# FibonacciDude/ContrastiveProsthetics

Measured on AMD Instinct MI355X. Metric: sEMG windows/sec contrastive step, 12-ch Ninapro, 1/2/4/8 MI355X, higher is better.
Workload: dtype bf16; 1 GPU; synthetic 12-ch sEMG, 41-class one-hot, batch 4096 groups/GPU (167936 windows/GPU/step), stock BN (--no_adabn), dp_emg=0.0635, d_e=16, random-init weights; global_batch_groups=4096, parallelism=dp1, loss=reference per-group loss, tile_schedule=static

## Files before the change

contrastiveprosthetics_amd/csrc/api.hip:

```cpp
#include <hip/hip_runtime.h>
#include <cstdio>
#include <cmath>

#include "../../include/cpnative.h"
#include "common.cuh"
#include "gemm_nt.cuh"
#include "gemm_nt256p.cuh"
#include "gemm_ws.cuh"
#include "gemm_tn.cuh"
#include "gemm_tn256.cuh"
#include "kernels_misc.cuh"
#include "conv_kernels.cuh"
#include "head.cuh"
#include "optim.cuh"
#include "eval.cuh"
#include "preprocess.cuh"
#include "glove.cuh"
#include "fp8.cuh"
#include "small.cuh"
#include "online.cuh"
#include "online_adapt.cuh"
#include "online_multi.cuh"

static thread_local char g_err[512] = "";
// ... 266 lines not shown
    return 0;
}

extern "C" int cp_gather_oob_count(uint32_t* count_out, int32_t reset, void* stream) {
    if (!count_out) return fail(CP_ERR_ARG, "cp_gather_oob_count args");
    unsigned int* ctr = nullptr;
    CK(hipGetSymbolAddress((void**)&ctr, HIP_SYMBOL(g_gather_oob)));
    CK(hipMemcpyAsync(count_out, ctr, sizeof(uint32_t), hipMemcpyDeviceToDevice, (hipStream_t)stream));
    if (reset) CK(hipMemsetAsync(ctr, 0, sizeof(uint32_t), (hipStream_t)stream));
    return 0;
}

#define CAP_BDA16 512
#define CAP_BDA8 512
#define CAP_BRB16 512
#define CAP_BRB8 512
static inline int grid_rows(int64_t rows, int rows_per_block, int cap) {
    int64_t g = (rows + rows_per_block - 1) / rows_per_block;
    return (int)(g > cap ? cap : (g < 1 ? 1 : g));
}

template <typename T> static inline int fc_bm() { return sizeof(T) == 2 ? 256 : 128; }
template <typename T, int EPI>
static inline hipError_t launch_fc_gemm(const GemmNTArgs& a, hipStream_t st, int* stat_rows = nullptr, bool dyn_schedule = false) {
    if (stat_rows) *stat_rows = (int)((a.M + fc_bm<T>() - 1) / fc_bm<T>());
    if constexpr (sizeof(T) == 2) {
        const bool dyn = dyn_schedule, ws_ok = !dyn;
        if (EPI == EPI_FWD && a.K == WS_K && a.lda == WS_K && a.relu && ws_ok) return launch_gemm_ws(a, st, stat_rows);
        if (EPI == EPI_FWD && a.K == WSK_K && a.lda == WSK_K && a.F == 512 && a.relu && ws_ok) return launch_gemm_ws16n(a, st, stat_rows);
        if (EPI == EPI_FWD || (a.R == nullptr && a.dp_thresh == 0)) return launch_gemm_nt256p<EPI>(a, st, stat_rows, dyn);
        if (EPI == EPI_DGRAD && a.R != nullptr && a.K == WS_K && a.lda == WS_K && ws_ok) return launch_gemm_wsd_bn(a, st, stat_rows);
        if constexpr (EPI == EPI_DGRAD)
            return a.coef ? launch_gemm_nt256p<EPI_DGRAD_BN>(a, st, stat_rows, dyn) : launch_gemm_nt256p<EPI_DGRAD_ST>(a, st, stat_rows, dyn);
        return hipErrorInvalidValue;
    } else {
        return launch_gemm_nt<T, 128, 128, ALOAD_PLAIN, EPI>(a, st);
    }
}

template <typename T>
static inline int conv_grid(int64_t n_windows) {
    const int64_t strips = (n_windows + CONV_WPB - 1) / CONV_WPB;
    const int64_t cap = sizeof(T) == 2 ? 512 : 256;
    return (int)(strips < cap ? strips : cap);
}

struct PreReduce {
    const float* partials;
    float* scratch;
    hipStream_t st;
    const float* operator()(int& nrows, int W, int direct_rows = FIN_DIRECT_ROWS) const {
        if (nrows <= direct_rows) return partials;
        hipLaunchKernelGGL(reduce_rows_kernel, dim3(W / 64, REDUCE_SLICES), dim3(256), 0, st, partials, nrows, W, scratch);
        nrows = REDUCE_SLICES;
        return scratch;
    }
};

static int sync_row(const cp_config* c, const float* pp, int nrows, int width, unsigned char* base, const WS& w, hipStream_t st,
                    const float** glob, const float** local, const int* unscale_exp = nullptr) {
    float* loc = (float*)(base + w.sync_loc);
    float* glo = (float*)(base + w.sync_glob);
    if (width > 2 * 768) return fail(CP_ERR_ARG, "sync_row width");
    hipLaunchKernelGGL(colsum_finalize_kernel, dim3(FIN_GRID(width)), dim3(FIN_THREADS), 0, st, pp, nrows, width, loc, unscale_exp, width / 2);
    CKL("colsum_finalize_kernel(sync)");
    CK(hipMemcpyAsync(glo, loc, (size_t)width * 4, hipMemcpyDeviceToDevice, st));
    if (int e = c->stats_allreduce(c->stats_user, glo, width, st)) return fail(e, "the statistics all-reduce hook failed");
    *glob = glo;
    if (local) *local = loc;
    return 0;
}

template <typename T>
static int encoder_forward_t(const cp_config* c, const cp_params* p, const cp_bn_buffers* bn, const float* x,
                             unsigned char* base, const WS& w, float* z, hipStream_t st) {
    using D = DT<T>;
    const int64_t N = c->n_windows, R12 = N * 12;
    const bool batch_stats = c->training || c->adabn;
    const bool have_running = bn && bn->running_mean[0] && bn->running_var[0];
    if (!batch_stats && !have_running) return fail(CP_ERR_ARG, "eval with stock BN needs running statistics");
    const int upd = (c->training && !c->adabn && have_running) ? 1 : 0;
    const bool drop = c->training && c->dp_emg > 0.f;
    float* partials = (float*)(base + w.partials);
    auto act = [&](int l) { return (T*)(base + w.act[l]); };
    auto stats = [&](int l) { return (float*)(base + w.stats[l]); };
    auto finalize = [&](int l, int nrows, double count) -> int {
        if (!batch_stats) return 0;
        ProfScope ps(CP_K_BN_FINALIZE, st);
        const int C = kLayerC[l];
        const PreReduce pre{partials, (float*)(base + w.partials2), st};
        const float* pp = batch_stats ? pre(nrows, 2 * C) : partials;
        if (batch_stats && c->stats_allreduce) {
            if (int e = sync_row(c, pp, nrows, 2 * C, base, w, st, &pp, nullptr)) return e;
            nrows = 1;
            count *= c->stats_world;
        }
        hipLaunchKernelGGL(bn_finalize_kernel, dim3(FIN_GRID(C)), dim3(FIN_THREADS), 0, st, pp, nrows, count, p->bn_g[l], p->bn_b[l],
                           have_running ? bn->running_mean[l] : nullptr, have_running ? bn->running_var[l] : nullptr, upd,
                           batch_stats ? 0 : 1, c->bn_momentum, c->bn_eps, stats(l), C);
        hipError_t e = hipGetLastError();
        return e == hipSuccess ? 0 : fail((int)e, "bn_finalize_kernel");
    };

    {
        ProfScope ps(CP_K_PREP, st);
        hipLaunchKernelGGL((prep_conv2_kernel<T>), dim3(48), dim3(256), 0, st, p->conv2_w, (T*)(base + w.wc2_f), (T*)(base + w.wc2_d));
        CKL("prep_conv2_kernel");
        if (!batch_stats) {
            BnRunningAll ra{};
            for (int l = 0; l < CP_N_BN; ++l) {
                ra.gamma[l] = p->bn_g[l]; ra.beta[l] = p->bn_b[l]; ra.mean[l] = bn->running_mean[l]; ra.var[l] = bn->running_var[l];
                ra.stats[l] = stats(l); ra.C[l] = kLayerC[l];
            }
            ra.eps = c->bn_eps;
            hipLaunchKernelGGL(bn_running_stats_kernel, dim3(CP_N_BN), dim3(512), 0, st, ra);
            CKL("bn_running_stats_kernel");
            FoldBnBatch fb{};
            for (int i = 0; i < CP_N_FC; ++i) {
                const int Lp = 1 + i;
                fb.job[i] = FoldBnJob{p->fc_w[i], p->fc_b[i], stats(Lp) + 2 * kLayerC[Lp], stats(Lp) + 3 * kLayerC[Lp], base + w.wfc[i],
                                      (float*)(base + w.bfc[i]), 512, fcK(i), i == 0 ? 1 : 0, 512};
            }
            fb.job[CP_N_FC] = FoldBnJob{p->last_w, nullptr, stats(8) + 2 * 512, stats(8) + 3 * 512, base + w.wlast, (float*)(base + w.blast), CP_D_E, 512, 0, 32};
            hipLaunchKernelGGL((fold_linear_batch_kernel<T>), dim3(512, CP_N_FC + 1), dim3(256), 0, st, fb);
            CKL("fold_linear_batch_kernel");
        }
        if (drop) {
            FoldBatch fb{};
            for (int q = 0; q < 3; ++q)
                fb.job[q] = FoldJob{p->fc_w[4 + q], p->fc_b[4 + q], base + w.wfc[4 + q], (float*)(base + w.bfc[4 + q]), 512, 512, 512};
            fb.job[3] = FoldJob{p->last_w, nullptr, base + w.wlast, (float*)(base + w.blast), CP_D_E, 512, 32};
            hipLaunchKernelGGL((fold_copy_batch_kernel<T>), dim3(512, 4), dim3(256), 0, st, fb);
            CKL("fold_copy_batch_kernel");
        }
    }
    {
        constexpr int RPP = 256 / (64 / D::EPC);
        const int64_t need = (N + RPP - 1) / RPP, passes = (need + 2047) / 2048;
        const int g = (int)((need + passes - 1) / passes);
        if (batch_stats) {
            ProfScope ps(CP_K_CONV1_FWD, st);
            hipLaunchKernelGGL((conv1_stats_kernel<T>), dim3(g), dim3(256), 0, st, x, p->conv1_w, p->conv1_b, partials, R12);
            CKL("conv1_stats_kernel");
        }
        if (int e = finalize(0, g, (double)R12)) return e;
    }
    {
        ConvArgs ca{};
        ca.x = x; ca.w1 = p->conv1_w; ca.b1 = p->conv1_b; ca.stats1 = stats(0);
        ca.wc = base + w.wc2_f; ca.bias2 = p->conv2_b; ca.out = act(1); ca.partials = batch_stats ? partials : nullptr; ca.n_windows = N;
        const int g = conv_grid<T>(N);
        {
            ProfScope ps(CP_K_CONV2_FWD, st);
            hipLaunchKernelGGL((conv2_strip_kernel<T, 0>), dim3(g), dim3(256), 0, st, ca);
            CKL("conv2_strip_kernel<fwd>");
        }
        if (int e = finalize(1, g, (double)R12)) return e;
    }
    for (int i = 0; i < CP_N_FC; ++i) {
        const int L = 2 + i, Lp = L - 1, K = fcK(i);
        const T* A = act(Lp);
        const float *s = stats(Lp) + 2 * kLayerC[Lp], *t = stats(Lp) + 3 * kLayerC[Lp];
        if (drop && Lp >= 5) {
            T* u = (T*)(base + w.u[Lp - 5]);
            ProfScope ps(CP_K_DROPOUT, st);
            hipLaunchKernelGGL((bn_dropout_apply_kernel<T>), dim3(grid_rows(N, 256 / (512 / D::EPC), CAP_BDA16)), dim3(256), 0, st,
                               act(Lp), stats(Lp), u, N, 512, dp_thresh(c->dp_emg), dp_key(c, Lp), dp_inv_keep(c->dp_emg), dp_salt(c));
            CKL("bn_dropout_apply_kernel");
            A = u; s = nullptr; t = nullptr;
        }
        if (!(drop && Lp >= 5) && batch_stats) {
            ProfScope ps(CP_K_FOLD, st);
            hipLaunchKernelGGL((fold_linear_kernel<T>), dim3(512), dim3(256), 0, st, p->fc_w[i], p->fc_b[i], s, t,
                               (T*)(base + w.wfc[i]), (float*)(base + w.bfc[i]), 512, K, i == 0 ? 1 : 0);
            CKL("fold_linear_kernel");
        }
        GemmNTArgs a{};
        a.A = A; a.lda = K; a.M = N; a.K = K;
        a.W = base + w.wfc[i]; a.F = 512;
        a.C = act(L); a.ldc = 512; a.bias = (float*)(base + w.bfc[i]); a.relu = 1;
        a.partials = (batch_stats || sizeof(T) != 2 || dyn_tiles(c)) ? partials : nullptr;
        int nrows = 0;
        {
            const bool ws = sizeof(T) == 2 && K == WS_K && !dyn_tiles(c);
            ProfScope ps(ws ? CP_K_FC_FWD_WS : CP_K_FC_FWD, st);
            CK((launch_fc_gemm<T, EPI_FWD>(a, st, &nrows, dyn_tiles(c))));
        }
        if (int e = finalize(L, nrows, (double)N)) return e;
    }
    {
        const int Lp = 8;
        const T* A = act(Lp);
        const float *s = stats(Lp) + 2 * 512, *t = stats(Lp) + 3 * 512;
        if (!drop && batch_stats) {
            ProfScope ps(CP_K_FOLD, st);
            hipLaunchKernelGGL((fold_linear_kernel<T>), dim3(32), dim3(256), 0, st, p->last_w, (const float*)nullptr, s, t,
                               (T*)(base + w.wlast), (float*)(base + w.blast), CP_D_E, 512, 0);
            CKL("fold_linear_kernel(last)");
        }
        GemmNTArgs a{};
        a.A = A; a.lda = 512; a.M = N; a.K = 512;
        a.W = base + w.wlast; a.F = 32;
        a.C = z; a.ldc = CP_D_E; a.f_valid = CP_D_E; a.bias = (float*)(base + w.blast);
        {
            ProfScope ps(CP_K_PROJ_FWD, st);
            if (drop) {
                a.a_scale = stats(Lp) + 2 * 512; a.a_shift = stats(Lp) + 3 * 512;
                a.dp_thresh = dp_thresh(c->dp_emg); a.dp_key = dp_key(c, Lp); a.dp_inv_keep = dp_inv_keep(c->dp_emg); a.dp_salt = dp_salt(c);
                CK((launch_gemm_nt<T, 128, 32, ALOAD_BNDROP, EPI_PLAIN_F32>(a, st)));
            } else {
                CK((launch_gemm_nt<T, 128, 32, ALOAD_PLAIN, EPI_PLAIN_F32>(a, st)));
            }
        }
    }
    return 0;
}


static int encoder_forward_fp8(const cp_config* c, const cp_params* p, const cp_bn_buffers* bn, const float* x,
                               unsigned char* base, const WS& w, float* z, hipStream_t st) {
    using T = bf16_t;
    using D = DT<T>;
    const int64_t N = c->n_windows, R12 = N * 12;
    const bool batch_stats = c->training || c->adabn;
    const bool have_running = bn && bn->running_mean[0] && bn->running_var[0];
    if (!batch_stats && !have_running) return fail(CP_ERR_ARG, "eval with stock BN needs running statistics");
    const int upd = (c->training && !c->adabn && have_running) ? 1 : 0;
    const bool drop = c->training && c->dp_emg > 0.f;
    float* partials = (float*)(base + w.partials);
    Fp8State* fs = (Fp8State*)(base + w.f8state);
    auto stats = [&](int l) { return (float*)(base + w.stats[l]); };
    auto finalize = [&](int l, int nrows, double count, const int* unscale) -> int {
        if (!batch_stats) return 0;
        ProfScope ps(CP_K_BN_FINALIZE, st);
        const int C = kLayerC[l];
        const PreReduce pre{partials, (float*)(base + w.partials2), st};
        const float* pp = batch_stats ? pre(nrows, 2 * C) : partials;
        if (batch_stats && c->stats_allreduce) {
            if (int e = sync_row(c, pp, nrows, 2 * C, base, w, st, &pp, nullptr, unscale)) return e;
            nrows = 1;
            count *= c->stats_world;
            unscale = nullptr;
        }
        hipLaunchKernelGGL(bn_finalize_kernel, dim3(FIN_GRID(C)), dim3(FIN_THREADS), 0, st, pp, nrows, count, p->bn_g[l], p->bn_b[l],
                           have_running ? bn->running_mean[l] : nullptr, have_running ? bn->running_var[l] : nullptr, upd,
                           batch_stats ? 0 : 1, c->bn_momentum, c->bn_eps, stats(l), C, unscale);
        hipError_t e = hipGetLastError();
        return e == hipSuccess ? 0 : fail((int)e, "bn_finalize_kernel");
    };
    {
        ProfScope ps(CP_K_PREP, st);
        hipLaunchKernelGGL(fp8_update_scales_kernel, dim3(1), dim3(64), 0, st, fs, N);
        hipLaunchKernelGGL((prep_conv2_kernel<T>), dim3(48), dim3(256), 0, st, p->conv2_w, (T*)(base + w.wc2_f), (T*)(base + w.wc2_d));
        if (!batch_stats) {
            BnRunningAll ra{};
            for (int l = 0; l < CP_N_BN; ++l) {
                ra.gamma[l] = p->bn_g[l]; ra.beta[l] = p->bn_b[l]; ra.mean[l] = bn->running_mean[l]; ra.var[l] = bn->running_var[l];
                ra.stats[l] = stats(l); ra.C[l] = kLayerC[l];
            }
            ra.eps = c->bn_eps;
            hipLaunchKernelGGL(bn_running_stats_kernel, dim3(CP_N_BN), dim3(512), 0, st, ra);
        }
        if (batch_stats && drop) {
            Fold8Batch fb{};
            for (int i = 4; i < CP_N_FC; ++i)
                fb.job[i - 4] = Fold8Job{p->fc_w[i], p->fc_b[i], nullptr, nullptr, base + w.wfc8[i], base + w.wsc8[i],
                                         (float*)(base + w.bfc[i]), fcK(i), 0, F8_T_U + (i - 4), F8_T_ACT + 2 + i};
            hipLaunchKernelGGL(fold_linear8_batch_kernel, dim3(512, CP_N_FC - 4), dim3(256), 0, st, fb, (const Fp8State*)fs);
        }
        CKL("prep kernels (fp8)");
    }
    {
        constexpr int RPP = 256 / (64 / D::EPC);
        const int64_t need = (N + RPP - 1) / RPP, passes = (need + 2047) / 2048;
        const int g = (int)((need + passes - 1) / passes);
        if (batch_stats) {
            ProfScope ps(CP_K_CONV1_FWD, st);
            hipLaunchKernelGGL((conv1_stats_kernel<T>), dim3(g), dim3(256), 0, st, x, p->conv1_w, p->conv1_b, partials, R12);
            CKL("conv1_stats_kernel");
        }
        if (int e = finalize(0, g, (double)R12, nullptr)) return e;
    }
    {
        ConvArgs ca{};
        ca.x = x; ca.w1 = p->conv1_w; ca.b1 = p->conv1_b; ca.stats1 = stats(0);
        ca.wc = base + w.wc2_f; ca.bias2 = p->conv2_b; ca.out = nullptr; ca.partials = batch_stats ? partials : nullptr; ca.n_windows = N;
        ca.out8 = base + w.act8[1]; ca.out_exp = &fs->e[F8_T_ACT + 1]; ca.out_amax = &fs->amax[F8_T_ACT + 1];
        const int g = conv_grid<T>(N);
        {
            ProfScope ps(CP_K_CONV2_FWD, st);
            hipLaunchKernelGGL((conv2_strip_kernel<T, 0>), dim3(g), dim3(256), 0, st, ca);
            CKL("conv2_strip_kernel<fwd, e4m3>");
        }
        if (int e = finalize(1, g, (double)R12, nullptr)) return e;
    }
    if (!batch_stats) {
        ProfScope ps(CP_K_FOLD, st);
        Fold8Batch fb{};
        for (int i = 0; i < CP_N_FC; ++i) {
            const int Lp = 1 + i;
            fb.job[i] = Fold8Job{p->fc_w[i], p->fc_b[i], stats(Lp) + 2 * kLayerC[Lp], stats(Lp) + 3 * kLayerC[Lp], base + w.wfc8[i], base + w.wsc8[i],
                                 (float*)(base + w.bfc[i]), fcK(i), i == 0 ? 1 : 0, F8_T_ACT + Lp, F8_T_ACT + 2 + i};
        }
        hipLaunchKernelGGL(fold_linear8_batch_kernel, dim3(512, CP_N_FC), dim3(256), 0, st, fb, (const Fp8State*)fs);
        CKL("fold_linear8_batch_kernel");
    }
    for (int i = 0; i < CP_N_FC; ++i) {
// ... 2120 lines not shown
```

contrastiveprosthetics_amd/csrc/conv_kernels.cuh:

```cuda
#pragma once
#include <type_traits>
#include "common.cuh"
#include "gemm_tn.cuh"

#define CONV_WPB 16
#define CONV_ROWS (CONV_WPB * 12)
#define CONV_IMG_ROWS (CONV_WPB * 14)

struct ConvArgs {
    const float* x;
    const float* w1;
    const float* b1;
    const float* stats1;
    const void* wc;
    const float* bias2;
    const void* gin;
    const int* gin_exp;
    const float* coef;
    void* out;
    uint8_t* out8;
    const int* out_exp;
    uint32_t* out_amax;
    float* partials;
    int64_t n_windows;
    SmBN bn1;
    long long* acc_out;
    const float* bn2_rows;
    int bn2_nr;
    const void* r2;
    const float* stats2;
    float* dgamma2;
    float* dbeta2;
    float* gcols3;
    const float* rows1;
    int rows1_nr;
    float* dgamma1;
    float* dbeta1;
};

__device__ __forceinline__ void conv_bn_bwd_coef(const float* __restrict__ rows, int nr, int nfold, const float* __restrict__ stats, double count,
                                                 float* ca, float* cb, float* cz, double (*red)[4][64], bool writer, float* dgamma, float* dbeta) {
    const int tid = threadIdx.x, c = tid & 63, part = tid >> 6, W = nfold * 64;
    double s1 = 0, s2 = 0;
    const int total = nr * nfold;
    int i = part;
    for (; i + 28 < total; i += 32) {
        float v1[8], v2[8];
#pragma unroll
        for (int u = 0; u < 8; ++u) {
            const int k = i + 4 * u, rw = k / nfold, f = k % nfold;
            v1[u] = rows[((int64_t)rw * 2 + 0) * W + f * 64 + c];
            v2[u] = rows[((int64_t)rw * 2 + 1) * W + f * 64 + c];
        }
#pragma unroll
        for (int u = 0; u < 8; ++u) { s1 += (double)v1[u]; s2 += (double)v2[u]; }
    }
    for (; i < total; i += 4) {
        const int rw = i / nfold, f = i % nfold;
        s1 += (double)rows[((int64_t)rw * 2 + 0) * W + f * 64 + c];
        s2 += (double)rows[((int64_t)rw * 2 + 1) * W + f * 64 + c];
    }
    red[0][part][c] = s1;
    red[1][part][c] = s2;
    __syncthreads();
    if (tid < 64) {
        s1 = (red[0][0][c] + red[0][1][c]) + (red[0][2][c] + red[0][3][c]);
        s2 = (red[1][0][c] + red[1][1][c]) + (red[1][2][c] + red[1][3][c]);
        const double mean = stats[c], invstd = stats[64 + c], sc = stats[128 + c];
        const double dot = (s2 - mean * s1) * invstd;
        const double c1 = s1 / count, c2 = dot / count;
        ca[c] = (float)sc;
        cb[c] = (float)(-sc * invstd * c2);
        cz[c] = (float)(-sc * (c1 - mean * invstd * c2));
        if (writer) { dgamma[c] = (float)dot; dbeta[c] = (float)s1; }
    }
    __syncthreads();
}

template <typename T> struct ConvGeo {
    using D = DT<T>;
    static constexpr int EPC = D::EPC;
    static constexpr int CPR = 64 / EPC;
    static constexpr int ROWB = 64 * (int)sizeof(T);
    static constexpr int RPP = 256 / CPR;
    static constexpr int WPITCH = 192 * (int)sizeof(T) + 16;
    static constexpr int CPITCH = ROWB + 16;
    __device__ static __forceinline__ int swz(int row) {
        const int d = row - 2 * (row / 14);
        return sizeof(T) == 2 ? ((d >> 1) & 7) : (d & 15);
    }
    __device__ static __forceinline__ int img_off(int row, int chunk) { return row * ROWB + ((chunk ^ swz(row)) << 4); }
};

template <typename T>
__device__ __forceinline__ void conv1_chunk_vals(float xm, float x0, float xp, const float (*wt)[3], const float* bs, float* out) {
    using D = DT<T>;
    const f32x2_t xm2 = {xm, xm}, x02 = {x0, x0}, xp2 = {xp, xp};
#pragma unroll
    for (int e = 0; e < D::EPC; e += 2) {
        f32x2_t y = {bs[e], bs[e + 1]};
        y = __builtin_elementwise_fma((f32x2_t){wt[e][0], wt[e + 1][0]}, xm2, y);
        y = __builtin_elementwise_fma((f32x2_t){wt[e][1], wt[e + 1][1]}, x02, y);
        y = __builtin_elementwise_fma((f32x2_t){wt[e][2], wt[e + 1][2]}, xp2, y);
        if constexpr (sizeof(T) == 2) {
            const uint32_t pk = cvt_pk_bf16<true>(y.x, y.y);
            out[e] = __uint_as_float(pk << 16);
            out[e + 1] = __uint_as_float(pk & 0xffff0000u);
        } else {
            out[e] = fmaxf(y.x, 0.f);
            out[e + 1] = fmaxf(y.y, 0.f);
        }
    }
}
template <typename T>
__device__ __forceinline__ void conv1_chunk_row(const float* xr, int w, const float (*wt)[3], const float* bs, float* out) {
    const float x0 = xr[w];
    const float xl = xr[w > 0 ? w - 1 : 0];
    const float xh = xr[w < 11 ? w + 1 : 11];
    conv1_chunk_vals<T>(w > 0 ? xl : 0.f, x0, w < 11 ? xh : 0.f, wt, bs, out);
}
template <typename T>
__device__ __forceinline__ void conv1_chunk(const float* __restrict__ x, int64_t win, int w, const float (*wt)[3],
                                            const float* bs, float* out) {
    conv1_chunk_row<T>(x + win * 12, w, wt, bs, out);
}

template <typename T>
__global__ __launch_bounds__(256) void conv1_stats_kernel(const float* __restrict__ x, const float* __restrict__ w,
                                                          const float* __restrict__ bias, float* __restrict__ partials,
                                                          int64_t rows, long long* __restrict__ acc = nullptr) {
    using G = ConvGeo<T>;
    constexpr int EPC = G::EPC, CPR = G::CPR, RPP = G::RPP;
    __shared__ float red[2][RPP][64];
    const int tid = threadIdx.x, cc = tid % CPR, rr = tid / CPR;
    float wt[EPC][3], bs[EPC];
    f32x2_t s1[EPC / 2], s2[EPC / 2];
#pragma unroll
    for (int e = 0; e < EPC; ++e) {
#pragma unroll
        for (int k = 0; k < 3; ++k) wt[e][k] = w[(cc * EPC + e) * 9 + 3 + k];
        bs[e] = bias[cc * EPC + e];
    }
#pragma unroll
    for (int k = 0; k < EPC / 2; ++k) s1[k] = s2[k] = (f32x2_t){0.f, 0.f};
    const int64_t nwin = rows / 12;
    for (int64_t win = (int64_t)blockIdx.x * RPP + rr; win < nwin; win += (int64_t)gridDim.x * RPP) {
        float xv[12];
#pragma unroll
        for (int q = 0; q < 3; ++q) {
            const float4 t = *(const float4*)(x + win * 12 + 4 * q);
            xv[4 * q] = t.x; xv[4 * q + 1] = t.y; xv[4 * q + 2] = t.z; xv[4 * q + 3] = t.w;
        }
#pragma unroll
        for (int w = 0; w < 12; ++w) {
            float v[EPC];
            conv1_chunk_vals<T>(w > 0 ? xv[w - 1] : 0.f, xv[w], w < 11 ? xv[w + 1] : 0.f, wt, bs, v);
// ... 106 lines not shown
    auto prefetch_g = [&](int64_t strip) {
        if constexpr (MODE == 1) {
#pragma unroll
            for (int it = 0; it < NITG; ++it) {
                const int ir = rr + it * RPP;
                const int nl = ir / 14, wp = ir % 14;
                const int64_t win = strip * CONV_WPB + nl;
                const bool ok = strip < nstrips && wp >= 1 && wp <= 12 && win < a.n_windows;
                pg[it] = *(const uint4*)((const T*)a.gin + ((ok ? win : 0) * 12 + (ok ? wp - 1 : 0)) * 64 + cc * EPC);
            }
        }
    };
    prefetch_g(blockIdx.x);
    __syncthreads();
    for (int64_t strip = blockIdx.x; strip < nstrips; strip += gridDim.x) {
        const int64_t win0 = strip * CONV_WPB;
        const float x_next = MODE == 0 ? load_x(strip + gridDim.x) : 0.f;
        const float* xcur = xs[MODE == 0 ? xb : 0];
        {
            constexpr int NIT = CONV_IMG_ROWS / RPP;
            uint4 v[NIT];
#pragma unroll
            for (int it = 0; it < NIT; ++it) {
                const int ir = rr + it * RPP;
                const int nl = ir / 14, wp = ir % 14;
                const int64_t win = win0 + nl;
                const bool ok = wp >= 1 && wp <= 12 && win < a.n_windows;
                const int64_t winc = ok ? win : 0;
                const int wpos = ok ? wp - 1 : 0;
                if constexpr (MODE == 0) {
                    float t[EPC];
                    conv1_chunk_row<T>(xcur + nl * 12, wpos, wt, bs, t);
#pragma unroll
                    for (int e = 0; e < EPC; ++e) t[e] = fmaf(t[e], sc[e], sh[e]);
                    v[it] = D::pack(t);
                } else {
                    v[it] = pg[it];
                }
                if (!ok) v[it] = make_uint4(0, 0, 0, 0);
            }
#pragma unroll
            for (int it = 0; it < NIT; ++it) *(uint4*)(img + G::img_off(rr + it * RPP, cc)) = v[it];
        }
        __syncthreads();
        prefetch_g(strip + gridDim.x);
        f32x16 acc[3];
#pragma unroll
        for (int j = 0; j < 3; ++j)
#pragma unroll
            for (int g = 0; g < 16; ++g) acc[j][g] = 0.f;
        int ir0[3];
#pragma unroll
        for (int j = 0; j < 3; ++j) {
            const int ml = (st0 + j) * 32 + r;
            ir0[j] = (ml / 12) * 14 + (ml % 12);
        }
#pragma unroll
        for (int ks = 0; ks < NKS; ++ks) {
            const int tap = ks / KS_PER_TAP, chunk = (ks % KS_PER_TAP) * 2 + h;
            const uint4 fw = *(const uint4*)(Wl + (ft * 32 + r) * WPITCH + ks * 32 + h * 16);
#pragma unroll
            for (int j = 0; j < 3; ++j) {
                const uint4 fs = *(const uint4*)(img + G::img_off(ir0[j] + tap, chunk));
                mma_chunk<T>(fw, fs, acc[j]);
            }
        }
        if (MODE == 0 && tid < CONV_WPB * 12) xs[xb ^ 1][tid] = x_next;
        __syncthreads();
#pragma unroll
        for (int j = 0; j < 3; ++j) {
            const int srow = (st0 + j) * 32 + r;
#pragma unroll
            for (int q = 0; q < 4; ++q) {
                const int fl = ft * 32 + 8 * q + 4 * h;
                f32x2_t v0 = {acc[j][4 * q], acc[j][4 * q + 1]}, v1 = {acc[j][4 * q + 2], acc[j][4 * q + 3]};
                if constexpr (MODE == 0) {
                    v0 += (f32x2_t){b2v[q][0], b2v[q][1]};
                    v1 += (f32x2_t){b2v[q][2], b2v[q][3]};
                }
                unsigned char* dst = Cs + srow * CPITCH + fl * (int)sizeof(T);
                if constexpr (sizeof(T) == 2) {
                    *(uint2*)dst = make_uint2(cvt_pk_bf16<MODE == 0>(v0.x, v0.y), cvt_pk_bf16<MODE == 0>(v1.x, v1.y));
                } else {
                    if constexpr (MODE == 0) { v0 = __builtin_elementwise_max(v0, (f32x2_t){0.f, 0.f}); v1 = __builtin_elementwise_max(v1, (f32x2_t){0.f, 0.f}); }
                    *(float4*)dst = make_float4(v0.x, v0.y, v1.x, v1.y);
                }
            }
        }
        __syncthreads();
#pragma unroll
        for (int p = 0; p < CONV_ROWS / RPP; ++p) {
            const int row = rr + p * RPP;
            const int64_t m = win0 * 12 + row;
            const bool ok = m < total_rows;
            const int64_t mc = ok ? m : 0;
            const uint4 c = *(const uint4*)(Cs + row * CPITCH + cc * 16);
            float v[EPC];
            D::unpack(ok ? c : make_uint4(0, 0, 0, 0), v);
            if constexpr (MODE == 0) {
                if (want_sums) {
#pragma unroll
                    for (int k = 0; k < EPC / 2; ++k) {
                        const f32x2_t vp = {v[2 * k], v[2 * k + 1]};
                        s1[k] += vp;
                        s2[k] = __builtin_elementwise_fma(vp, vp, s2[k]);
                    }
                }
            } else {
                float r1[EPC];
                conv1_chunk<T>(a.x, mc / 12, (int)(mc % 12), wt, bs, r1);
#pragma unroll
                for (int k = 0; k < EPC / 2; ++k) {
                    const f32x2_t vp = {v[2 * k], v[2 * k + 1]}, rp = {r1[2 * k], r1[2 * k + 1]};
                    s1[k] += vp;
                    s2[k] = __builtin_elementwise_fma(vp, rp, s2[k]);
                }
            }
            if constexpr (MODE == 0 && sizeof(T) == 2) {
                if (a.out8 != nullptr) {
                    float w8[EPC];
#pragma unroll
                    for (int e = 0; e < EPC; ++e) { w8[e] = v[e] * out_scale; out_max = fmaxf(out_max, w8[e]); }
                    int p0 = __builtin_amdgcn_cvt_pk_fp8_f32(w8[0], w8[1], 0, false), p1 = __builtin_amdgcn_cvt_pk_fp8_f32(w8[4], w8[5], 0, false);
                    p0 = __builtin_amdgcn_cvt_pk_fp8_f32(w8[2], w8[3], p0, true);
                    p1 = __builtin_amdgcn_cvt_pk_fp8_f32(w8[6], w8[7], p1, true);
                    if (ok) *(uint2*)(a.out8 + m * 64 + cc * EPC) = make_uint2((uint32_t)p0, (uint32_t)p1);
                    continue;
                }
            }
            if (ok) *(uint4*)((T*)a.out + m * 64 + cc * EPC) = c;
        }
        __syncthreads();
        xb ^= 1;
    }
    if constexpr (MODE == 0 && sizeof(T) == 2) {
        if (a.out8 != nullptr) {
            out_max = wave_max(out_max);
            if ((tid & 63) == 0 && out_max > 0.f && __float_as_uint(out_max) > __hip_atomic_load(a.out_amax, __ATOMIC_RELAXED, __HIP_MEMORY_SCOPE_AGENT))
                atomicMax(a.out_amax, __float_as_uint(out_max));
        }
    }
#pragma unroll
    for (int e = 0; e < EPC; ++e) { red[(0 * RPP + rr) * 64 + cc * EPC + e] = s1[e / 2][e & 1]; red[(1 * RPP + rr) * 64 + cc * EPC + e] = s2[e / 2][e & 1]; }
    __syncthreads();
    if (tid < 128 && want_sums) {
        const int which = tid >> 6, c = tid & 63;
        float s = 0.f;
        for (int q = 0; q < RPP; ++q) s += red[(which * RPP + q) * 64 + c];
        if (MODE == 0 && a.acc_out != nullptr) sm_acc_add(a.acc_out + which * 64 + c, s, SM_ACT_SHIFT);
        else a.partials[((int64_t)blockIdx.x * 2 + which) * 64 + c] = s;
    }
}

#define CONV_WG_WPB 8
#define CONV_WG_IMG (CONV_WG_WPB * 14)
template <typename T, bool G8 = false, bool BN2 = false>
__global__ __launch_bounds__(256, BN2 ? 1 : 2) void conv2_wgrad_kernel(ConvArgs a) {
    static_assert(!G8 || sizeof(T) == 2, "e5m2 gradients are expanded into a bf16 image");
    static_assert(!(G8 && BN2), "the small-batch form reads T gradients");
    using GV = std::conditional_t<G8, uint2, uint4>;
    using D = DT<T>;
    using G = ConvGeo<T>;
    constexpr int EPC = G::EPC, CPR = G::CPR, RPP = G::RPP, KSTEP = D::KSTEP;
    constexpr int PITCH = TNPitch<T, 64>::value;
    constexpr int ROWS = CONV_WG_IMG + 2;
    constexpr int NIT = (CONV_WG_IMG + RPP - 1) / RPP;
    __shared__ __attribute__((aligned(16))) unsigned char smem[2 * ROWS * PITCH];
    unsigned char* Xi = smem;
    unsigned char* Yi = smem + ROWS * PITCH;
    const int tid = threadIdx.x, lane = tid & 63, wave = tid >> 6;
    const int cc = tid % CPR, rr = tid / CPR;
    const int ot = wave & 1, it = wave >> 1;
    const int64_t nstrips = (a.n_windows + CONV_WG_WPB - 1) / CONV_WG_WPB;

    float wt[EPC][3], bs[EPC], sc[EPC], sh[EPC];
#pragma unroll
    for (int e = 0; e < EPC; ++e) {
        const int c = cc * EPC + e;
#pragma unroll
        for (int k = 0; k < 3; ++k) wt[e][k] = a.w1[c * 9 + 3 + k];
        bs[e] = a.b1[c];
        sc[e] = a.stats1 ? a.stats1[2 * 64 + c] : 1.f;
        sh[e] = a.stats1 ? a.stats1[3 * 64 + c] : 0.f;
    }
    f32x16 acc[3];
#pragma unroll
    for (int j = 0; j < 3; ++j)
#pragma unroll
        for (int g = 0; g < 16; ++g) acc[j][g] = 0.f;
    uint4 xr2[BN2 ? NIT : 1];
    float c2a[BN2 ? EPC : 1], c2b[BN2 ? EPC : 1], c2z[BN2 ? EPC : 1], cs_all[BN2 ? EPC : 1], cs_first[BN2 ? EPC : 1], cs_last[BN2 ? EPC : 1];
    if constexpr (BN2) {
        __shared__ float ca_s[64], cb_s[64], cz_s[64];
        conv_bn_bwd_coef(a.bn2_rows, a.bn2_nr, 12, a.stats2, (double)a.n_windows * 12, ca_s, cb_s, cz_s, (double (*)[4][64])smem, blockIdx.x == 0,
                         a.dgamma2, a.dbeta2);
#pragma unroll
        for (int e = 0; e < EPC; ++e) {
            c2a[e] = ca_s[cc * EPC + e]; c2b[e] = cb_s[cc * EPC + e]; c2z[e] = cz_s[cc * EPC + e];
            cs_all[e] = cs_first[e] = cs_last[e] = 0.f;
        }
        __syncthreads();
    }
    if (rr == 0) {
        *(uint4*)(Xi + 0 * PITCH + cc * 16) = make_uint4(0, 0, 0, 0);
        *(uint4*)(Xi + (ROWS - 1) * PITCH + cc * 16) = make_uint4(0, 0, 0, 0);
        *(uint4*)(Yi + 0 * PITCH + cc * 16) = make_uint4(0, 0, 0, 0);
        *(uint4*)(Yi + (ROWS - 1) * PITCH + cc * 16) = make_uint4(0, 0, 0, 0);
    }
    GV xg[NIT];
    float xr[NIT][3];
    float gd = 1.f;
    if constexpr (G8) gd = f8_exp2i(-*a.gin_exp);
    auto prefetch = [&](int64_t strip) {
        const int64_t win0 = strip * CONV_WG_WPB;
#pragma unroll
        for (int q = 0; q < NIT; ++q) {
            const int ir = rr + q * RPP;
            const int nl = ir / 14, wp = ir % 14;
            const int64_t win = win0 + nl;
            const bool ok = strip < nstrips && ir < CONV_WG_IMG && wp >= 1 && wp <= 12 && win < a.n_windows;
            const int64_t winc = ok ? win : 0;
            const int wpos = ok ? wp - 1 : 0;
            xg[q] = *(const GV*)((const unsigned char*)a.gin + ((winc * 12 + wpos) * 64 + cc * EPC) * (int64_t)sizeof(GV) / EPC);
            if constexpr (BN2) xr2[q] = *(const uint4*)((const T*)a.r2 + (winc * 12 + wpos) * 64 + cc * EPC);
            const float* xw = a.x + winc * 12;
            xr[q][0] = xw[wpos > 0 ? wpos - 1 : 0];
            xr[q][1] = xw[wpos];
            xr[q][2] = xw[wpos < 11 ? wpos + 1 : 11];
        }
    };
    prefetch(blockIdx.x);
    for (int64_t strip = blockIdx.x; strip < nstrips; strip += gridDim.x) {
        const int64_t win0 = strip * CONV_WG_WPB;
        {
#pragma unroll
            for (int q = 0; q < NIT; ++q) {
                const int ir = rr + q * RPP;
                const int nl = ir / 14, wp = ir % 14;
                const bool ok = ir < CONV_WG_IMG && wp >= 1 && wp <= 12 && win0 + nl < a.n_windows;
                const int wpos = ok ? wp - 1 : 0;
                float t[EPC];
                conv1_chunk_vals<T>(wpos > 0 ? xr[q][0] : 0.f, xr[q][1], wpos < 11 ? xr[q][2] : 0.f, wt, bs, t);
                if (a.stats1 != nullptr) {
#pragma unroll
                    for (int e = 0; e < EPC; ++e) t[e] = fmaf(t[e], sc[e], sh[e]);
                }
                uint4 yv = D::pack(t);
                uint4 xv;
                if constexpr (G8) xv = f8_chunk5_to_bf16(xg[q], gd);
                else xv = xg[q];
                if constexpr (BN2) {
                    float gv[EPC], rv[EPC];
                    D::unpack(xv, gv);
                    D::unpack(xr2[q], rv);
#pragma unroll
                    for (int e = 0; e < EPC; ++e) gv[e] = rv[e] > 0.f ? fmaf(c2a[e], gv[e], fmaf(c2b[e], rv[e], c2z[e])) : 0.f;
                    xv = D::pack(gv);
                    if (ok) {
                        *(uint4*)((T*)const_cast<void*>(a.gin) + ((win0 + nl) * 12 + wpos) * 64 + cc * EPC) = xv;
                        D::unpack(xv, gv);
#pragma unroll
                        for (int e = 0; e < EPC; ++e) {
                            cs_all[e] += gv[e];
                            cs_first[e] += wpos == 0 ? gv[e] : 0.f;
                            cs_last[e] += wpos == 11 ? gv[e] : 0.f;
                        }
                    }
                }
                if (!ok) { xv = make_uint4(0, 0, 0, 0); yv = make_uint4(0, 0, 0, 0); }
                if (ir < CONV_WG_IMG) {
                    *(uint4*)(Xi + (ir + 1) * PITCH + cc * 16) = xv;
                    *(uint4*)(Yi + (ir + 1) * PITCH + cc * 16) = yv;
                }
            }
        }
        __syncthreads();
        prefetch(strip + gridDim.x);
#pragma unroll
        for (int k0 = 0; k0 < CONV_WG_IMG; k0 += KSTEP) {
            uint4 fy;
            if constexpr (sizeof(T) == 2) fy = tn_frag_bf16<PITCH>(Yi, k0 + 1, it * 32, lane);
            else fy = tn_frag_f32<PITCH>(Yi, k0 + 1, it * 32, lane);
#pragma unroll
            for (int tap = 0; tap < 3; ++tap) {
                uint4 fx;
                if constexpr (sizeof(T) == 2) fx = tn_frag_bf16<PITCH>(Xi, k0 + 2 - tap, ot * 32, lane);
                else fx = tn_frag_f32<PITCH>(Xi, k0 + 2 - tap, ot * 32, lane);
                mma_chunk<T>(fx, fy, acc[tap]);
            }
        }
        __syncthreads();
    }
    float* slab = a.partials + (int64_t)blockIdx.x * 64 * 192;
    const int r = lane & 31, h = lane >> 5;
#pragma unroll
    for (int tap = 0; tap < 3; ++tap) {
        const int q = tap * 64 + it * 32 + r;
#pragma unroll
        for (int g = 0; g < 16; ++g) {
            const int p = ot * 32 + (g & 3) + 8 * (g >> 2) + 4 * h;
            slab[p * 192 + q] = acc[tap][g];
        }
    }
    if constexpr (BN2) {
        float* red = (float*)smem;
        static_assert(2 * ROWS * PITCH >= 3 * RPP * 64 * 4, "the column-sum reduction reuses the image region");
// ... 168 lines not shown
```

Before: 47.39 million windows/s.

## Add software-pipelined conv2 forward kernel double-buffering the conv1 image build

Adds a new 16-bit conv2 forward kernel that loops persistently over strips. It builds the next strip's conv1+BN image into a second LDS buffer while the MFMA chains for the current strip run, and uses sched_group_barrier hints to interleave the two. Weights stay in registers, batch-stat sums are kept in registers and reduced once at the end, and outputs are stored through buffer stores. The aim is to hide LDS image construction and global loads behind matrix work, at the cost of higher register and LDS pressure and a more complex schedule.

```diff
diff --git a/contrastiveprosthetics_amd/csrc/api.hip b/contrastiveprosthetics_amd/csrc/api.hip
--- a/contrastiveprosthetics_amd/csrc/api.hip
+++ b/contrastiveprosthetics_amd/csrc/api.hip
@@ -442,7 +442,12 @@
         const int g = conv_grid<T>(N);
         {
             ProfScope ps(CP_K_CONV2_FWD, st);
-            hipLaunchKernelGGL((conv2_strip_kernel<T, 0>), dim3(g), dim3(256), 0, st, ca);
+            if constexpr (sizeof(T) == 2) {
+                if (batch_stats) hipLaunchKernelGGL((conv2_fwd_pipe_kernel<T, true>), dim3(g), dim3(256), 0, st, ca);
+                else hipLaunchKernelGGL((conv2_fwd_pipe_kernel<T, false>), dim3(g), dim3(256), 0, st, ca);
+            } else {
+                hipLaunchKernelGGL((conv2_strip_kernel<T, 0>), dim3(g), dim3(256), 0, st, ca);
+            }
             CKL("conv2_strip_kernel<fwd>");
         }
         if (int e = finalize(1, g, (double)R12)) return e;
diff --git a/contrastiveprosthetics_amd/csrc/conv_kernels.cuh b/contrastiveprosthetics_amd/csrc/conv_kernels.cuh
--- a/contrastiveprosthetics_amd/csrc/conv_kernels.cuh
+++ b/contrastiveprosthetics_amd/csrc/conv_kernels.cuh
@@ -2,6 +2,7 @@
 #include <type_traits>
 #include "common.cuh"
 #include "gemm_tn.cuh"
+#include "gemm_ws.cuh"
 
 #define CONV_WPB 16
 #define CONV_ROWS (CONV_WPB * 12)
@@ -414,6 +415,195 @@
     }
 }
 
+typedef __attribute__((ext_vector_type(2))) unsigned int u32x2_t;
+template <typename T, bool SUMS>
+__global__ __launch_bounds__(256, 2) void conv2_fwd_pipe_kernel(ConvArgs a) {
+    static_assert(sizeof(T) == 2, "the pipelined forward is the 16-bit large-batch form");
+    using D = DT<T>;
+    using G = ConvGeo<T>;
+    constexpr int EPC = G::EPC, CPR = G::CPR, ROWB = G::ROWB, RPP = G::RPP;
+    constexpr int KSTEP = D::KSTEP, KS_PER_TAP = 64 / KSTEP, NKS = 3 * KS_PER_TAP;
+    constexpr int IMG_BYTES = CONV_IMG_ROWS * ROWB, NIT = CONV_IMG_ROWS / RPP, XN = CONV_WPB * 12;
+    static_assert(2 * IMG_BYTES >= 2 * 64 * 64 * 4, "the end-of-kernel reduction reuses the image buffers");
+    __shared__ __attribute__((aligned(128))) unsigned char smem[2 * IMG_BYTES];
+    static_assert(IMG_BYTES % 128 == 0, "fragment addresses: the k chunk is XORed into bits 5-6 behind the buffer's offset");
+    constexpr int XP = CONV_WPB * 16 + 4;
+    __shared__ float xs[2][XP];
+    __shared__ __attribute__((aligned(16))) float b2s[64];
+    const int tid = threadIdx.x, lane = tid & 63, wave = tid >> 6;
+    const int r = lane & 31, h = lane >> 5;
+    const int cc = tid % CPR, rr = tid / CPR;
+    const int ft = wave & 1, st0 = 3 * (wave >> 1);
+    const int64_t nstrips = (a.n_windows + CONV_WPB - 1) / CONV_WPB;
+    const int64_t total_rows = a.n_windows * 12;
+    const int64_t grid = gridDim.x;
+
+    uint4 wf[NKS];
+#pragma unroll
+    for (int ks = 0; ks < NKS; ++ks) wf[ks] = *(const uint4*)((const T*)a.wc + (ft * 32 + r) * 192 + ks * KSTEP + h * EPC);
+    float wt[EPC][3], bs[EPC];
+    f32x2_t sc[EPC / 2], sh[EPC / 2];
+#pragma unroll
+    for (int e = 0; e < EPC; ++e) {
+        const int c = cc * EPC + e;
+#pragma unroll
+        for (int k = 0; k < 3; ++k) wt[e][k] = a.w1[c * 9 + 3 + k];
+        bs[e] = a.b1[c];
+        sc[e / 2][e & 1] = a.stats1 ? a.stats1[2 * 64 + c] : 1.f;
+        sh[e / 2][e & 1] = a.stats1 ? a.stats1[3 * 64 + c] : 0.f;
+    }
+    if (tid < 64) b2s[tid] = a.bias2[tid];
+    f32x2_t s1[2][4], s2[2][4];
+#pragma unroll
+    for (int pr = 0; pr < 2; ++pr)
+#pragma unroll
+        for (int k = 0; k < 4; ++k) s1[pr][k] = s2[pr][k] = (f32x2_t){0.f, 0.f};
+    int imeta[NIT];
+#pragma unroll
+    for (int it = 0; it < NIT; ++it) {
+        const int ir = rr + it * RPP, wp = ir % 14;
+        imeta[it] = (ir / 14) * 16 + ((wp >= 1 && wp <= 12) ? wp - 1 : 15);
+    }
+    int fa[3][3];
+#pragma unroll
+    for (int j = 0; j < 3; ++j) {
+        const int ml = (st0 + j) * 32 + r;
+#pragma unroll
+        for (int tap = 0; tap < 3; ++tap) fa[j][tap] = G::img_off((ml / 12) * 14 + (ml % 12) + tap, h);
+    }
+    auto load_x = [&](int64_t strip) {
+        const int64_t i = strip * XN + tid;
+        return (tid < XN && strip < nstrips && i < total_rows) ? a.x[i] : 0.f;
+    };
+    auto build_row = [&](unsigned char* img, const float* xsrc, int64_t win0, int it) {
+        const int nl = imeta[it] >> 4;
+        const bool ok = (imeta[it] & 15) != 15 && win0 + nl < a.n_windows;
+        const float* xw = xsrc + imeta[it];
+        float t[EPC];
+        conv1_chunk_vals<T>(xw[0], xw[1], xw[2], wt, bs, t);
+        const uint32_t keep = ok ? ~0u : 0u;
+        uint32_t pk[EPC / 2];
+#pragma unroll
+        for (int k = 0; k < EPC / 2; ++k) {
+            const f32x2_t u = __builtin_elementwise_fma((f32x2_t){t[2 * k], t[2 * k + 1]}, sc[k], sh[k]);
+            pk[k] = pack2bf(u.x, u.y) & keep;
+        }
+        const int ir = rr + it * RPP;
+        *(uint4*)(img + ir * ROWB + ((cc ^ (((ir - 2 * nl) >> 1) & 7)) << 4)) = make_uint4(pk[0], pk[1], pk[2], pk[3]);
+    };
+    auto chain = [&](int img_off, int j, f32x16& acc) {
+#pragma unroll
+        for (int q = 0; q < 4; ++q) {
+            const float4 b2 = *(const float4*)(b2s + ft * 32 + 8 * q + 4 * h);
+            acc[4 * q] = b2.x; acc[4 * q + 1] = b2.y; acc[4 * q + 2] = b2.z; acc[4 * q + 3] = b2.w;
+        }
+#pragma unroll
+        for (int tap = 0; tap < 3; ++tap) {
+            const int ab = fa[j][tap] + img_off;
+#pragma unroll
+            for (int kq = 0; kq < KS_PER_TAP; ++kq) {
+                const uint4 fs = *(const uint4*)(smem + (ab ^ (kq << 5)));
+                mma_chunk<T>(wf[tap * KS_PER_TAP + kq], fs, acc);
+            }
+        }
+    };
+    auto epilogue = [&](const f32x16& acc, int j, int64_t m0) {
+        const int srow = (st0 + j) * 32 + r;
+        const int64_t left = total_rows - m0;
+        const bool ok = srow < left;
+        const int nrows = left < CONV_ROWS ? (int)left : CONV_ROWS;
+        uint2 pk[4];
+#pragma unroll
+        for (int q = 0; q < 4; ++q) {
+            pk[q] = make_uint2(cvt_pk_bf16<true>(acc[4 * q], acc[4 * q + 1]), cvt_pk_bf16<true>(acc[4 * q + 2], acc[4 * q + 3]));
+        }
+#pragma unroll
+        for (int pr = 0; pr < 2; ++pr) {
+            const auto sx = __builtin_amdgcn_permlane32_swap(pk[2 * pr].x, pk[2 * pr + 1].x, false, false);
+            const auto sy = __builtin_amdgcn_permlane32_swap(pk[2 * pr].y, pk[2 * pr + 1].y, false, false);
+            const u32x4_t c = {sx[0], sy[0], sx[1], sy[1]};
+            const int f0 = ft * 32 + 16 * pr + 8 * h;
+            float v[EPC];
+            D::unpack(ok ? make_uint4(c.x, c.y, c.z, c.w) : make_uint4(0, 0, 0, 0), v);
+            if constexpr (SUMS) {
+#pragma unroll
+                for (int k = 0; k < EPC / 2; ++k) {
+                    const f32x2_t vp = {v[2 * k], v[2 * k + 1]};
+                    s1[pr][k] += vp;
+                    s2[pr][k] = __builtin_elementwise_fma(vp, vp, s2[pr][k]);
+                }
+            }
+            const auto rsrc = __builtin_amdgcn_make_buffer_rsrc((T*)a.out + m0 * 64, 0, nrows * ROWB, 0x00020000);
+            store_b128_settled(c, rsrc, (uint32_t)(srow * ROWB + f0 * 2), 0, 0);
+        }
+    };
+
+    auto interleave = [&]() {
+        __builtin_amdgcn_sched_group_barrier(0x100, 2, 0);
+#pragma unroll
+        for (int i = 0; i < NKS; ++i) {
+            __builtin_amdgcn_sched_group_barrier(0x008, 1, 0);
+            __builtin_amdgcn_sched_group_barrier(0x100, 1, 0);
+        }
+        __builtin_amdgcn_sched_barrier(0);
+    };
+    const int xslot = (tid / 12) * 16 + 1 + tid % 12;
+    for (int i = tid; i < 2 * XP; i += 256) (&xs[0][0])[i] = 0.f;
+    __syncthreads();
+    if (tid < XN) { xs[0][xslot] = load_x(blockIdx.x); xs[1][xslot] = load_x(blockIdx.x + grid); }
+    __syncthreads();
+#pragma unroll
+    for (int it = 0; it < NIT; ++it) build_row(smem, xs[0], (int64_t)blockIdx.x * CONV_WPB, it);
+    __syncthreads();
+    int cur = 0;
+    for (int64_t strip = blockIdx.x; strip < nstrips; strip += grid) {
+        const int ic = cur * IMG_BYTES;
+        unsigned char* inx = smem + (cur ^ 1) * IMG_BYTES;
+        const float* xn = xs[cur ^ 1];
+        const int64_t m0 = strip * CONV_ROWS, win_n = (strip + grid) * CONV_WPB;
+        const float x_next = load_x(strip + 2 * grid);
+        f32x16 acc[3];
+        __builtin_amdgcn_sched_barrier(0);
+        chain(ic, 0, acc[0]);
+#pragma unroll
+        for (int it = 0; it < 3; ++it) build_row(inx, xn, win_n, it);
+        interleave();
+        chain(ic, 1, acc[1]);
+        epilogue(acc[0], 0, m0);
+#pragma unroll
+        for (int it = 3; it < 5; ++it) build_row(inx, xn, win_n, it);
+        interleave();
+        chain(ic, 2, acc[2]);
+        epilogue(acc[1], 1, m0);
+#pragma unroll
+        for (int it = 5; it < NIT; ++it) build_row(inx, xn, win_n, it);
+        interleave();
+        epilogue(acc[2], 2, m0);
+        if (tid < XN) xs[cur][xslot] = x_next;
+        __syncthreads();
+        cur ^= 1;
+    }
+    if constexpr (SUMS) {
+        float* red = (float*)smem;
+        const int slot = (wave >> 1) * 32 + r;
+#pragma unroll
+        for (int pr = 0; pr < 2; ++pr)
+#pragma unroll
+            for (int e = 0; e < EPC; ++e) {
+                const int f = ft * 32 + 16 * pr + 8 * h + e;
+                red[(0 * 64 + slot) * 64 + f] = s1[pr][e / 2][e & 1];
+                red[(1 * 64 + slot) * 64 + f] = s2[pr][e / 2][e & 1];
+            }
+        __syncthreads();
+        if (tid < 128) {
+            const int which = tid >> 6, c = tid & 63;
+            float s = 0.f;
+            for (int q = 0; q < 64; ++q) s += red[(which * 64 + q) * 64 + c];
+            a.partials[((int64_t)blockIdx.x * 2 + which) * 64 + c] = s;
+        }
+    }
+}
+
 #define CONV_WG_WPB 8
 #define CONV_WG_IMG (CONV_WG_WPB * 14)
 template <typename T, bool G8 = false, bool BN2 = false>
```

Result: no change. 47.55 million windows/s, median of 6 (+0.3%).
